# david-cortes/recometrics

Hardware: AMD Instinct MI355X
Metric: users/sec evaluated (all metrics, K=10) (higher is better)
Workload: dtype f32

## Files before the change

### recometrics_amd/_binding.py

```python
import ctypes as C
import os

import numpy as np

_LIB_PATH = os.environ.get("RECOMETRICS_HIP_LIB") or os.path.join(
    os.path.dirname(os.path.abspath(__file__)), "csrc", "librecometrics_hip.so")
_lib = None

METRIC_ORDER = ("p", "tp", "r", "ap", "tap", "ndcg", "hit", "rr", "roc", "pr")
OUTPUTS = tuple(name + ("_auc" if name in ("roc", "pr") else "_at_k") for name in METRIC_ORDER)

_vp, _i32, _i64, _u64, _sz, _ci = C.c_void_p, C.c_int32, C.c_int64, C.c_uint64, C.c_size_t, C.c_int
_FACTORS = (("A", _vp), ("lda", _sz), ("B", _vp), ("ldb", _sz), ("m", _i32), ("n", _i32), ("k", _i32))
_SCORES = (("S", _vp), ("lds", _sz), ("m", _i32), ("n", _i32))


def _csr(which, host, values=False):
    return ((("X%s_csr_p" % which, _vp), ("X%s_csr_i" % which, _vp)) + ((("X%s_csr" % which, _vp),) if values else ())
            + (() if host else (("nnz_" + which, _i64),)))


def _metrics(source, host):
    return (source + _csr("train", host) + _csr("test", host, values=True) + (("k_metrics", _i32), ("cumulative", _ci))
            + ((("break_ties_with_noise", _ci),) if source is _FACTORS else ()) + tuple((name, _vp) for name in OUTPUTS)
# ... 15 lines not shown
                       ("seed", _u64), ("result", C.POINTER(_vp)))}
_TYPED.update({"rm_" + request + source + form: pieces(params, host) for request, pieces in (("calc_metrics", _metrics), ("recommend", _lists))
               for source, params in (("", _FACTORS), ("_scores", _SCORES)) for form, host in (("", True), ("_dev", False))})
SIGNATURES = {name + suffix: (params, _ci) for name, params in _TYPED.items() for suffix in ("_f32", "_f64")}
SIGNATURES.update({
    "rm_has_openmp": ((), _ci), "rm_last_error": ((), C.c_char_p), "rm_device_count": ((), _ci), "rm_set_device": ((("device", _ci),), _ci),
    "rm_set_devices": ((("devices", C.POINTER(_i32)), ("n", _i32)), _ci), "rm_get_devices": ((("devices", C.POINTER(_i32)), ("cap", _i32)), _ci),
    "rm_request_interrupt": ((), None), "rm_get_timings": ((("out", C.POINTER(C.c_double)), ("n", _ci)), _ci), "rm_release_workspace": ((), _ci),
    "rm_debug_reload_switches": ((), None), "rm_debug_sweep_variants": ((("elem_bytes", _ci), ("out", C.POINTER(_ci)), ("cap", _ci)), _ci),
    "rm_debug_find_sweep": (tuple((name, _ci) for name in ("elem_bytes", "ng", "ngt", "auc", "dump", "lmode", "nsub", "spec"))
                            + (("out6", C.POINTER(_ci)),), _ci),
    "rm_debug_supported_ng": ((("elem_bytes", _ci), ("k", _ci)), _ci),
    "rm_debug_sweep_launched": ((("elem_bytes", _ci), ("counts", C.POINTER(_ci)), ("cap", _ci)), _ci), "rm_debug_sweep_launched_reset": ((), None),
    "rm_split_size": ((("result", _vp), ("which", _ci)), _i64), "rm_split_copy": ((("result", _vp), ("which", _ci), ("dst", _vp)), _ci),
    "rm_split_free": ((("result", _vp),), None), "rm_split_last_error": ((), C.c_char_p),
    "rm_csr_rows_sorted": ((("indptr", _vp), ("indices", _vp), ("m", _i32), ("nthreads", _i32)), _ci),
    "rm_csr_sort_rows": ((("indptr", _vp), ("indices", _vp), ("values", _vp), ("value_bytes", _i32), ("m", _i32), ("nthreads", _i32)), _ci),
})
EXPORTS = tuple(SIGNATURES)
HALF_KINDS = ("f16", "bf16")
HALF_SIGNATURES = {"rm_" + request + "_scores" + form + "_" + kind: (pieces(_SCORES, host), _ci)
                   for request, pieces in (("calc_metrics", _metrics), ("recommend", _lists)) for form, host in (("", True), ("_dev", False))
                   for kind in HALF_KINDS}
TEST_HOOKS = {"rm_debug_set_list_ids": ((("ids", C.POINTER(_i32)), ("m", _i32), ("K", _i32)), _ci)}


class HipLibraryMissing(ImportError):
    pass


def lib_path():
    return _LIB_PATH


def _declare(lib, names, table=None):
    for name in names:
        params, restype = (table or SIGNATURES)[name]
        fn = getattr(lib, name)
        fn.argtypes, fn.restype = [ctype for _, ctype in params], restype
    return lib


def load():
    global _lib
    if _lib is None:
        if not os.path.exists(_LIB_PATH):
            raise HipLibraryMissing(
# ... 91 lines not shown


def timings():
    lib = load()
    buf = (C.c_double * 11)()
    n = lib.rm_get_timings(buf, 11)
    keys = ("prep_ms", "sweep_ms", "finalize_ms", "device_ms", "sweep_launches", "item_splits", "sweep_blocks", "lds_bytes",
            "timed_slots", "total_slots", "split_reused")
    return {k: buf[i] for i, k in enumerate(keys[:n])}


def hinted_users():
    lib = load()
    buf = (C.c_double * 12)()
    return int(buf[11]) if lib.rm_get_timings(buf, 12) >= 12 else 0


def set_list_ids(ids):
    lib = load()
    ids = np.ascontiguousarray(ids, dtype=np.int32)
    rc = lib.rm_debug_set_list_ids(ids.ctypes.data_as(C.POINTER(_i32)), ids.shape[0], ids.shape[1])
    if rc:
        _raise(lib, rc)


def csr_rows_sorted(indptr, indices, nthreads=0):
    lib = _load_split()
    assert indptr.dtype == np.int32 and indices.dtype == np.int32
    rc = lib.rm_csr_rows_sorted(_p(indptr), _p(indices), indptr.shape[0] - 1, int(nthreads))
    if rc < 0:
        raise ValueError("rm_csr_rows_sorted: bad argument")
    return bool(rc)


def csr_sort_rows(indptr, indices, data, nthreads=0):
    lib = _load_split()
    assert indptr.dtype == np.int32 and indices.dtype == np.int32 and indices.flags.writeable
    vb = 0 if data is None else data.dtype.itemsize
    if vb not in (0, 4, 8):
        raise ValueError("values must be 4 or 8 bytes wide")
    rc = lib.rm_csr_sort_rows(_p(indptr), _p(indices), None if data is None else _p(data), vb, indptr.shape[0] - 1, int(nthreads))
    if rc:
        raise (MemoryError if rc == 3 else ValueError)("rm_csr_sort_rows failed (status %d)" % rc)


def _invoke(entry, dtype, **values):
# ... 181 lines not shown
```

### recometrics_amd/csrc/rm_device.hpp

```cpp
#pragma once
#include <hip/hip_runtime.h>
#include <stdint.h>

namespace rm {

constexpr int WAVE = 64;
constexpr int GROUP_USERS = 32;
constexpr int TILE_ITEMS = 64;
constexpr int SWEEP_THREADS = 512;
constexpr int GROUPS_PER_BLOCK = 4;
constexpr int POS_CHUNK = 63;
constexpr int MAX_J = 6;
constexpr int STREAM_CLASS = MAX_J + 1;
constexpr int N_CLASSES = MAX_J + 2;
constexpr int IDX_EMPTY = 0x7fffffff;
constexpr int HEAVY_NPOS = 256;
enum : int { LM_LDS = 0, LM_HBM = 1, LM_HBM_APPEND = 2 };
constexpr int WAIT_VMCNT0 = 0x0F70;

enum : int { UF_NAN = 1, UF_ONLY_NDCG = 2, UF_KLEQN = 4, UF_ACTIVE = 8, UF_SKIP = 16 };

enum : int { RQ_P = 1, RQ_TP = 2, RQ_R = 4, RQ_AP = 8, RQ_TAP = 16, RQ_NDCG = 32, RQ_HIT = 64, RQ_RR = 128, RQ_ROC = 256, RQ_PR = 512 };

template <class T> struct Entry { T s; int idx; };
typedef Entry<float> ListEntry;

template <class T> struct PartialStat {
    T vmax, vmin;
    unsigned long long rocsum;
    int has_nan; int pad;
};

struct Plan {
    int n_active;
    int n_slots;
    int n_groups;
    int jmax;
// ... 61 lines not shown
```

### recometrics_amd/csrc/rm_finalize.hpp

```cpp
#pragma once
#include "rm_device.hpp"
#include "rm_kernel_units.hpp"
#include <type_traits>

namespace rm {

constexpr int MAX_PARTS = 128;
constexpr int FIN_THREADS = 128;
constexpr int FIN_TOPV = 64;
template <class T> inline size_t finalize_lds_bytes(int K, int n_part) { return (sizeof(T) * (size_t)(K < FIN_TOPV ? K : FIN_TOPV) + 4 * (size_t)n_part) * FIN_THREADS; }

struct AucPart { unsigned long long sum_ranks; double s1, s2; int nvalid, pad; };

template <class T, class S> struct FinalArgs {
    int m, n, K, n_part, req, cumulative, noise, gu, n_slots;
    const int *slot_user, *slot_chunk;
    const int *train_p, *test_p, *test_i; const T *test_v;
    const int *flags, *user_nslots, *uslot_base, *slot_index;
    const int *gj; const long long *grow;
    const Entry<S> *pl; const PartialStat<S> *pst; const unsigned *hist; const S *pos_score;
    const int *pos_item_tab;
    AucPart *auc_part;
    T *heavy_topv;
    unsigned char *heavy_nan;
// ... 105 lines not shown
                const int pos = filled + __popcll(mk & ((1ull << lane) - 1ull));
                if (cand && pos < K) { L[pos].s = x; L[pos].idx = PI[i]; }
                filled += __popcll(mk);
            }
        }
    }
    #pragma unroll
    for (int d = 32; d >= 1; d >>= 1) {
        const S om = __shfl_xor(vmax, d), on = __shfl_xor(vmin, d);
        vmax = om > vmax ? om : vmax; vmin = on < vmin ? on : vmin;
        has_nan |= __shfl_xor(has_nan, d);
    }
    for (int i = (filled < K ? filled : K) + lane; i < K; i += WAVE) { L[i].s = -(S)INFINITY; L[i].idx = IDX_EMPTY; }
    if (lane == 0) {
        PartialStat<S> ps;
        ps.vmax = vmax; ps.vmin = vmin; ps.rocsum = 0; ps.has_nan = has_nan; ps.pad = 0;
        ((PartialStat<S> *)a.pst)[(size_t)slot * NP + extra] = ps;
    }
}

constexpr int STREAM_RANK_THREADS = 256;
constexpr int STREAM_RANK_ITEMS = 128;
constexpr int STREAM_RANK_LDS = 20 * 1024;
template <class S, int ILP, int LV>
__device__ __forceinline__ void rank_streamed_lds(const S *row, long long i0, int ipt, int n, const int *pit, int P, int top_rt, int lgsb_rt,
                                                  unsigned tab_addr, unsigned hist_addr)
{
    const int top = LV ? (1 << LV) : top_rt;
    const int lgsb = LV ? 14 - LV : lgsb_rt;
    typedef __attribute__((address_space(3))) const S *LdsS;
    typedef __attribute__((address_space(3))) unsigned *LdsU;
    const unsigned sb = 1u << lgsb;
    auto load_batch = [&](int it, S (&x)[ILP]) {
        #pragma unroll
        for (int q = 0; q < ILP; q++) {
            const long long item = i0 + (long long)(it + q) * STREAM_RANK_THREADS + threadIdx.x;
            x[q] = row[item < n ? item : n - 1];
        }
    };
    S nxt[ILP];
    load_batch(0, nxt);
    for (int it = 0; it < ipt; it += ILP) {
        S v[ILP]; unsigned o[ILP];
        #pragma unroll
        for (int q = 0; q < ILP; q++) {
            const long long item = i0 + (long long)(it + q) * STREAM_RANK_THREADS + threadIdx.x;
// ... 42 lines not shown
        const S ps = live ? a.spos_score[te0 + j] : (S)0;
        const bool valid = live && !(isinf(ps) && ps > 0);
        const unsigned long long vm = __ballot(valid);
        const unsigned long long rank = above + incl + 1;
        const int myidx = nvalid + __popcll(vm & ((1ull << lane) - 1ull)) + 1;
        const double term = valid ? (double)myidx / (double)rank : 0.;
        unsigned long long rs = valid ? rank : 0ull;
        #pragma unroll
        for (int dd = 32; dd >= 1; dd >>= 1) {
            const unsigned lo32 = (unsigned)__shfl_xor((int)(unsigned)rs, dd), hi32 = (unsigned)__shfl_xor((int)(unsigned)(rs >> 32), dd);
            rs += ((unsigned long long)hi32 << 32) | lo32;
        }
        sum_ranks += rs;
        for (unsigned long long mm = vm; mm; mm &= mm - 1) s2 += lane_bcast<double>(term, __ffsll((long long)mm) - 1);
        if (a.rank_sorted && valid) a.rank_sorted[te0 + j] = (long long)rank;
        const int last = (base < WAVE ? base : WAVE) - 1;
        above += ((unsigned long long)(unsigned)__shfl((int)(unsigned)(incl >> 32), last) << 32) | (unsigned)__shfl((int)(unsigned)incl, last);
        nvalid += __popcll(vm);
    }
    if (lane == 0) { AucPart r; r.sum_ranks = sum_ranks; r.s1 = 0; r.s2 = s2; r.nvalid = nvalid; r.pad = 0; a.auc_part[slot] = r; }
}

template <class S>
__device__ __forceinline__ bool rank_block_walks(int fused_auc, int P)
{
    if (!(fused_auc & 1)) return false;
    constexpr int per = (int)sizeof(S) / 4;
    int top = 1;
    while (top <= P) top <<= 1;
    return (long long)top * per + P + 1 <= STREAM_RANK_LDS / 4;
}

#define RM_FCMP_LT(m, p, x) asm volatile("v_cmp_lt_f32 %0, %1, %2" : "=s"(m) : "v"(p), "v"(x))
#define RM_FCMP_LT_S(m, p, x) asm volatile("v_cmp_lt_f32 %0, %1, %2" : "=s"(m) : "s"(p), "v"(x))
#define RM_FSEL(d, a, b, m) asm volatile("v_cndmask_b32 %0, %1, %2, %3" : "=v"(d) : "v"(a), "v"(b), "s"(m))
template <int LV>
__device__ __forceinline__ void rank_streamed_fast(const float *row, int i0, int iters, const int *pit, int P, unsigned tab_addr, unsigned hist0_addr,
                                                   float piv_lo, float piv_root, float piv_hi)
{
    constexpr int ILP = 8;
    constexpr int LGSB = 14 - LV;
    constexpr unsigned SB = 1u << LGSB;
    constexpr unsigned Q = SB << (LV - 2);
    typedef __attribute__((address_space(3))) const float *LdsS;
    const float *src = row + i0 + (int)threadIdx.x;
    float nxt[ILP];
    #pragma unroll
    for (int q = 0; q < ILP; q++) nxt[q] = src[q * STREAM_RANK_THREADS];
    const unsigned a1 = tab_addr | Q, a2 = tab_addr | (2 * Q), a3 = tab_addr | (3 * Q);
    for (int it = 0; it < iters; it += ILP) {
        float v[ILP]; unsigned at[ILP];
        #pragma unroll
        for (int q = 0; q < ILP; q++) { v[q] = nxt[q]; at[q] = tab_addr; }
        src += ILP * STREAM_RANK_THREADS;
        if (it + ILP < iters) {
            #pragma unroll
            for (int q = 0; q < ILP; q++) nxt[q] = src[q * STREAM_RANK_THREADS];
        }
        unsigned long long mk0, mk1, mk2;
        #pragma unroll
        for (int i = 0; i < 3 * ILP + 2; i++) {
            if (i < 3 * ILP) {
                const float pv = i < ILP ? piv_lo : (i < 2 * ILP ? piv_root : piv_hi);
                if (i % 3 == 0) RM_FCMP_LT_S(mk0, pv, v[i % ILP]); else if (i % 3 == 1) RM_FCMP_LT_S(mk1, pv, v[i % ILP]); else RM_FCMP_LT_S(mk2, pv, v[i % ILP]);
// ... 27 lines not shown
        #pragma unroll
        for (int q = 0; q < ILP; q++) tie |= nx[q] == v[q];
        if (__any(tie)) {
            #pragma unroll
            for (int q = 0; q < ILP; q++) {
                if (nx[q] == v[q]) {
                    const int item = i0 + (it + q) * STREAM_RANK_THREADS + (int)threadIdx.x;
                    int l = (int)((at[q] - tab_addr) >> LGSB);
                    while (l < P && *(LdsS)(tab_addr + ((unsigned)l << LGSB)) == v[q] && pit[l] > item) l++;
                    at[q] = tab_addr + ((unsigned)l << LGSB);
                }
            }
        }
        const unsigned one = 1u;
        #pragma unroll
        for (int q = 0; q < ILP; q++) {
            const unsigned ha = hist0_addr + (((at[q] - tab_addr) >> LGSB) << 2);
            asm volatile("ds_add_u32 %0, %1" :: "v"(ha), "v"(one) : "memory");
        }
    }
    __builtin_amdgcn_s_waitcnt(0xC07F);
}

template <class T, class S>
__global__ __launch_bounds__(STREAM_RANK_THREADS) void k_rank_streamed(FinalArgs<T, S> a, int parts, int ipt, int row0)
{
    __shared__ __attribute__((aligned(16384))) char rk_smem[STREAM_RANK_LDS];
    const int d = row0 + blockIdx.x / parts, part = blockIdx.x % parts;
    const int slot = a.stream_slot0 + d;
    const int u = a.slot_user[slot];
    if (a.flags[u] & UF_ONLY_NDCG) return;
    const int te0 = a.test_p[u], P = a.test_p[u + 1] - te0;
    constexpr int WORDS = STREAM_RANK_LDS / 4;
    constexpr int per = (int)sizeof(S) / 4;
    int top = 1;
    while (top <= P) top <<= 1;
    int R = 0;
    if ((long long)top * per + P + 1 <= WORDS) { R = 1; while (R < 32 && (long long)top * 2 * R * per + P + 1 <= WORDS) R *= 2; }
    const int *pit = a.spos_item + te0;
    const S *row = a.stream_scores + (size_t)d * (size_t)a.stream_ld;
    const long long i0 = (long long)part * STREAM_RANK_THREADS * ipt;
    if (R > 0) {
        S *lds_s = (S *)rk_smem;
        unsigned *lds_h = (unsigned *)(rk_smem + sizeof(S) * (size_t)top * (size_t)R) + 1;
        for (int i = threadIdx.x; i < top * R; i += STREAM_RANK_THREADS) { const int e = i / R; lds_s[i] = e < P ? a.spos_score[te0 + e] : (S)INFINITY; }
        for (int i = threadIdx.x; i < P; i += STREAM_RANK_THREADS) lds_h[i] = 0u;
        __syncthreads();
        int lgsb = sizeof(S) == 4 ? 2 : 3;
        for (int r = R; r > 1; r >>= 1) lgsb++;
        const unsigned tab_addr = (unsigned)(size_t)(__attribute__((address_space(3))) char *)rk_smem + (unsigned)((threadIdx.x & (R - 1)) * sizeof(S));
        const unsigned hist_addr = (unsigned)(size_t)(__attribute__((address_space(3))) char *)lds_h;
        const bool full = (long long)top * R == 4096 / per;
        if (sizeof(S) == 4 && full && top >= 128 && top <= 1024 && !a.rank_generic) {
            const int inside = (int)((a.n - i0) / STREAM_RANK_THREADS);
            const int iters = inside <= 0 ? 0 : (inside < ipt ? inside : ipt) / 8 * 8;
            if (iters > 0) {
                const float *tabf = (const float *)lds_s;
                const float p_lo = tabf[(top / 4 - 1) * R], p_root = tabf[(top / 2 - 1) * R], p_hi = tabf[(3 * top / 4 - 1) * R];
                const float s_lo = __builtin_bit_cast(float, __builtin_amdgcn_readfirstlane(__builtin_bit_cast(int, p_lo)));
                const float s_root = __builtin_bit_cast(float, __builtin_amdgcn_readfirstlane(__builtin_bit_cast(int, p_root)));
                const float s_hi = __builtin_bit_cast(float, __builtin_amdgcn_readfirstlane(__builtin_bit_cast(int, p_hi)));
                const float *rowf = (const float *)row;
                const unsigned h0 = hist_addr - 4u;
                if (top == 128) rank_streamed_fast<7>(rowf, (int)i0, iters, pit, P, tab_addr, h0, s_lo, s_root, s_hi);
                else if (top == 256) rank_streamed_fast<8>(rowf, (int)i0, iters, pit, P, tab_addr, h0, s_lo, s_root, s_hi);
                else if (top == 512) rank_streamed_fast<9>(rowf, (int)i0, iters, pit, P, tab_addr, h0, s_lo, s_root, s_hi);
                else rank_streamed_fast<10>(rowf, (int)i0, iters, pit, P, tab_addr, h0, s_lo, s_root, s_hi);
            }
            if (iters < ipt) rank_streamed_lds<S, 8, 0>(row, i0 + (long long)iters * STREAM_RANK_THREADS, ipt - iters, a.n, pit, P, top, lgsb, tab_addr, hist_addr);
        } else
        if (full && top == 128) rank_streamed_lds<S, 8, 7>(row, i0, ipt, a.n, pit, P, top, lgsb, tab_addr, hist_addr);
        else if (full && top == 256) rank_streamed_lds<S, 8, 8>(row, i0, ipt, a.n, pit, P, top, lgsb, tab_addr, hist_addr);
        else if (full && top == 512) rank_streamed_lds<S, 8, 9>(row, i0, ipt, a.n, pit, P, top, lgsb, tab_addr, hist_addr);
        else if (full && top == 1024) rank_streamed_lds<S, 8, 10>(row, i0, ipt, a.n, pit, P, top, lgsb, tab_addr, hist_addr);
        else rank_streamed_lds<S, 8, 0>(row, i0, ipt, a.n, pit, P, top, lgsb, tab_addr, hist_addr);
        __syncthreads();
        if (parts == 1 && (a.fused_auc & 1)) {
            if (threadIdx.x < WAVE) {
                const bool own = (a.fused_auc & 2) != 0;
                const S *sp = a.spos_score + te0;
                auc_walk_streamed<T, S>(a, slot, te0, P, (int)threadIdx.x, [&](int j) {
                    unsigned c = lds_h[j];
                    if (own && j + 1 < P) { const S x = sp[j + 1]; c += (!(isinf(x) && x > 0) && x == x) ? 1u : 0u; }
                    return c;
                });
            }
            return;
        }
        for (int i = threadIdx.x; i < P; i += STREAM_RANK_THREADS) { const unsigned c = lds_h[i]; if (c) atomicAdd(&a.shist[te0 + i], c); }
    } else {
// ... 797 lines not shown
```

### recometrics_amd/csrc/rm_lib.hip

```cpp
#include <hip/hip_runtime.h>

#include <algorithm>
#include <array>
#include <cmath>
#include <cstdio>
#include <cstring>
#include <cstdlib>
#include <type_traits>
#include <atomic>
#include <chrono>
#include <condition_variable>
#include <csignal>
#include <functional>
#include <limits>
#include <map>
#include <memory>
#include <mutex>
#include <string>
#include <thread>
#include <vector>

#include "../../include/recometrics_hip.h"
#include "../../include/recometrics_hip_half.h"
#include "rm_device.hpp"
// ... 1024 lines not shown
            side.await(SIDE_CHECKS_DONE, stream); pos.await(POS_MAXIMA_DONE, stream);
            HIP_CHECK(hipMemcpyAsync(cx.pinned_plan, plan, sizeof(Plan), hipMemcpyDeviceToHost, stream));
            if (attempt == 0 && flat_early) {
                const hipStream_t sc = pos.fork(POS_SCORES_AFTER_COPY);
                if (c.scores) {
                    hipLaunchKernelGGL(k_test_masked, dim3(cdiv(m, TM_USERS)), dim3(256), 0, sc, m, c.test_p, c.test_i, c.train_p, c.train_i, ent_user, ent_masked, plan);
                    with_score_src<T>(c.s_type, [&](auto *src) {
                        typedef std::remove_cv_t<std::remove_pointer_t<decltype(src)>> Src;
                        hipLaunchKernelGGL((k_pos_scores_given<T, Src>), dim3(cdiv(c.nnz_test, 256)), dim3(256), 0, sc, pf, (const Src *)c.S, c.lds, (const int *)ent_user, (const unsigned char *)ent_masked);
                    });
                } else {
                hipLaunchKernelGGL(k_pos_scores_flat<T>, dim3(cdiv(c.nnz_test, POSF_WAVES * WAVE)), dim3(POSF_WAVES * WAVE), 0, sc, pf, ent_user);
                if (masked_from_bits) side.await(SIDE_ROWS_FOR_POS, sc);
                else hipLaunchKernelGGL(k_test_masked, dim3(cdiv(m, TM_USERS)), dim3(256), 0, sc, m, c.test_p, c.test_i, c.train_p, c.train_i, ent_user, ent_masked, plan);
                hipLaunchKernelGGL(k_pos_apply_masked<T>, dim3(cdiv(c.nnz_test, 256)), dim3(256), 0, sc, pf, ent_masked);
                }
                pos.mark(POS_SCORES_DONE);
            }
            RM_TRACE_POINT("run: plan chain + side kernels enqueued");
            HIP_CHECK(hipStreamSynchronize(stream));
            RM_TRACE_POINT("run: plan read back");
            hp = *cx.pinned_plan;
            throw_csr_defects(hp, c, cx);
            if (ca.allow_stream && !ca.force_stream && hp.class_count[STREAM_CLASS] > stream_cap && attempt == 0) {
                ca.allow_stream = 0; ca.check_ptr = 0; keepable = false;
                side.sync(); pos.sync();
                continue;
            }
            break;
        }
        if (!reused) throw_csr_defects(hp, c, cx);
        n_slots = hp.n_slots;
        n_stream = (want_auc || ext_topk) ? hp.class_count[STREAM_CLASS] : 0;
        stream_slot0 = n_stream > 0 ? hp.class_offset[STREAM_CLASS] : n_slots;
        if (!reused) check_nan = scores_may_overflow();
    }
    bool scores_may_overflow()
    {
        if (items_known) { hp.amax_b = cx.packed.amax_b; hp.nonfinite_b = cx.packed.nonfinite_b; }
        else { cx.packed.amax_b = hp.amax_b; cx.packed.nonfinite_b = hp.nonfinite_b; }
        double amax_a, amax_b;
        std::memcpy(&amax_a, &hp.amax_a, 8); std::memcpy(&amax_b, &hp.amax_b, 8);
        const double tmax = std::is_same<T, float>::value ? 3.0e38 : 1.0e308;
        if (c.scores) return false;
        return hp.nonfinite || hp.nonfinite_b || !((double)k * amax_a * 1.001 < tmax / std::max(amax_b, 1e-300));
    }

    bool make_split_key(SplitKey &key) const
    {
        std::memset(&key, 0, sizeof(SplitKey));
        if (g_sw.no_split_cache || !use_side || c.reco || c.scores || !c.plain() || c.items_tag != 0 || !c.test_p || m <= 0) return false;
        const void *arr[SPLIT_ARRAYS] = {c.train_p, c.train_i, c.test_p, c.test_i, c.test_v};
        const long long words[SPLIT_ARRAYS] = {(long long)m + 1, std::max<long long>(c.nnz_train, 0), (long long)m + 1, std::max<long long>(c.nnz_test, 0),
                                               c.test_v ? std::max<long long>(c.nnz_test, 0) * (long long)(sizeof(T) / 4) : 0};
        long long total = 0;
        for (int i = 0; i < SPLIT_ARRAYS; i++) { key.arr[i] = arr[i]; key.words[i] = words[i]; total += words[i]; }
// ... 301 lines not shown
    }

    void topk_rows()
    {
        HIP_CHECK(hipEventRecord(cx.ev[EV_PREP_END], stream));
        const void *kernel = nullptr;
        with_score_src<T>(c.s_type, [&](auto *src) {
            typedef std::remove_cv_t<std::remove_pointer_t<decltype(src)>> Src;
            RowTopkArgs<T, Src> ra{n, K, c.train_p, c.train_i, (const Src *)c.S, c.lds, c.topk_idx, c.topk_score, c.status};
            hipLaunchKernelGGL((k_topk_rows<T, Src>), dim3((unsigned)m), dim3(SCORE_ROW_THREADS), 0, stream, ra);
            kernel = (const void *)k_topk_rows<T, Src>;
        });
        HIP_CHECK(hipGetLastError());
        RM_TRACE_POINT("run: row top-K enqueued");
        HIP_CHECK(hipEventRecord(cx.ev[EV_SWEEP_END], stream));
        double *tm = cx.timings;
        hipFuncAttributes at{};
        HIP_CHECK(hipFuncGetAttributes(&at, kernel));
        tm[4] = 1; tm[5] = 1; tm[6] = m; tm[7] = (double)at.sharedSizeBytes;
        cx.timed_slots = hp.n_slots; cx.total_slots = hp.n_slots;
    }

    int stream_parts() const { return (int)cdiv(n, STREAM_RANK_THREADS * STREAM_RANK_ITEMS); }
    void rank_streamed_rows(int r0, int r1, hipStream_t st)
    {
        if (r1 <= r0) return;
        const int parts = stream_parts();
        const int ipt = ((int)cdiv(n, (long long)parts * STREAM_RANK_THREADS) + 7) / 8 * 8;
        hipLaunchKernelGGL((k_rank_streamed<T, T>), dim3((unsigned)((long long)(r1 - r0) * parts)), dim3(STREAM_RANK_THREADS), 0, st, fa, parts, ipt, r0);
    }
    void auc_streamed_rows(int r0, int r1, hipStream_t st)
    {
        if (r1 <= r0) return;
        hipLaunchKernelGGL((k_auc_streamed<T, T>), dim3(cdiv((long long)(r1 - r0) * WAVE, 256)), dim3(256), 0, st, fa, r0, r1);
    }
    void finalize_slots(int s0, int s1, size_t fin_lds)
    {
        if (s1 <= s0) return;
        fa.fin_slot0 = s0; fa.fin_slot1 = s1;
        hipLaunchKernelGGL((k_finalize<T, T>), dim3(cdiv(s1 - s0, FIN_THREADS)), dim3(FIN_THREADS), fin_lds, stream, fa);
    }

    void collect_lists()
    {
        if (!collect) return;
        fa.collected = 1;
        const char *gl = (const char *)glists;
        if (collect_capw(K, collect_g.lane_cap) == 512)
            hipLaunchKernelGGL((k_collect_topk<T, T, ThrT, 512>), dim3(collect_grid(cdiv(n_slots, 4))), dim3(256), 0, stream, fa, collect_g, gl, lane_cnt, (const ThrT *)thr_shared);
        else if (collect_capw(K, collect_g.lane_cap) == 1024)
            hipLaunchKernelGGL((k_collect_topk<T, T, ThrT, 1024>), dim3(collect_grid(cdiv(n_slots, 4))), dim3(256), 0, stream, fa, collect_g, gl, lane_cnt, (const ThrT *)thr_shared);
        else
// ... 15 lines not shown
        fa.n_part = g.n_part; fa.pl = pl; fa.pst = pst;
        fa.stream_slot0 = stream_slot0; fa.stream_scores = stream_scores; fa.stream_ld = stream_ld;
        collect_lists();
        select_lists();
        const bool merged_ready = n_slots > 0 && (collect || ext_topk);
        RecoArgs<T> ra{m, n, K, g.n_part, flags, uslot_base, slot_index, c.train_p, pl, pst, merged_ready ? merged : nullptr,
                       c.topk_idx, c.topk_score, c.status};
        const size_t lds = reco_lds_bytes<T>(g.n_part, merged_ready);
        if (lds > 48 * 1024) HIP_CHECK(hipFuncSetAttribute((const void *)k_finalize_reco<T>, hipFuncAttributeMaxDynamicSharedMemorySize, (int)lds));
        hipLaunchKernelGGL(k_finalize_reco<T>, dim3(cdiv(m, RECO_THREADS)), dim3(RECO_THREADS), lds, stream, ra);
        HIP_CHECK(hipGetLastError());
    }

    void finalize()
    {
        fa.n_part = g.n_part; fa.pl = pl; fa.pst = pst; fa.hist = hist; fa.pos_score = pos_score; fa.pos_item_tab = pos_item;
        fa.stream_slot0 = stream_slot0; fa.stream_scores = stream_scores; fa.stream_ld = stream_ld;
        fa.spos_score = spos_score; fa.spos_item = spos_item; fa.shist = shist;
        fa.rank_generic = (g_sw.rank_generic ? 1 : 0);
        const bool ranks_beside = use_side && n_slots > 0 && want_auc && n_stream > 0;
        bool auc_launch = true;
        if (stream_parts() == 1 && !g_sw.no_fused_auc) {
            fa.fused_auc = 1 | (g.mask_test ? 2 : 0);
            long long top = 1;
            while (top <= hp.max_npos) top <<= 1;
            auc_launch = ext_topk || !(top * (long long)(sizeof(T) / 4) + hp.max_npos + 1 <= STREAM_RANK_LDS / 4);
        }
        hipStream_t rank_stream = stream;
        if (ranks_beside) { rank_stream = side.fork(SIDE_FORK); rank_streamed_rows(0, n_stream, rank_stream); }
        if (g.mask_test) {
            if (n_slots > stream_slot0)
                hipLaunchKernelGGL((k_merge_positives<T, T>), dim3(cdiv(n_slots - stream_slot0, MERGE_WAVES)), dim3(MERGE_WAVES * WAVE), 0, stream, fa, g.n_part - 1, stream_slot0);
            if (ranks_beside && auc_launch) rank_stream = side.fork(SIDE_MERGED);
        }
        if (ranks_beside && auc_launch) auc_streamed_rows(0, n_stream, rank_stream);
        hipLaunchKernelGGL((k_finalize_skipped<T, T>), dim3(cdiv(m, 256)), dim3(256), 0, stream, fa);
        if (side.marked(SIDE_TOP_VALUES)) side.await(SIDE_TOP_VALUES, stream);
        collect_lists();
        select_lists();
        if (n_slots > 0) {
            if (want_auc) {
                if (n_stream > 0 && !ranks_beside) { rank_streamed_rows(0, n_stream, stream); if (auc_launch) auc_streamed_rows(0, n_stream, stream); }
                if (stream_slot0 > 0) hipLaunchKernelGGL((k_auc_slots<T, T>), dim3(cdiv(stream_slot0, 256)), dim3(256), 0, stream, fa);
            }
            const size_t fin_lds = finalize_lds_bytes<T>(K, g.n_part);
            HIP_CHECK(hipFuncSetAttribute((const void *)k_finalize<T, T>, hipFuncAttributeMaxDynamicSharedMemorySize, (int)fin_lds));
            fa.auc_defer_slot0 = n_slots;
            if (ranks_beside && (req & (RQ_ROC | RQ_PR)) && !g_sw.no_defer_auc) {
                fa.auc_defer_slot0 = stream_slot0;
                finalize_slots(0, n_slots, fin_lds);
                side.join(SIDE_JOIN);
                hipLaunchKernelGGL((k_finalize_auc<T, T>), dim3(cdiv(n_slots - stream_slot0, 256)), dim3(256), 0, stream, fa);
            } else if (ranks_beside) {
                finalize_slots(0, stream_slot0, fin_lds);
                side.join(SIDE_JOIN);
                finalize_slots(stream_slot0, n_slots, fin_lds);
            } else finalize_slots(0, n_slots, fin_lds);
        }
        HIP_CHECK(hipGetLastError());
    }

    void export_ranks()
    {
        if (c.topk_idx && !c.reco)
            hipLaunchKernelGGL(k_export_rank<T>, dim3(cdiv((long long)m * K, 256)), dim3(256), 0, stream, m, K, merged, c.topk_idx, c.topk_score, flags);
// ... 1254 lines not shown
{
    return elem_bytes == 4   ? debug_find_sweep<SweepArgs>(ng, ngt, auc, dump, lmode, nsub, spec, out6)
           : elem_bytes == 8 ? debug_find_sweep<Sweep64Args>(ng, ngt, auc, dump, lmode, nsub, spec, out6) : -1;
}
extern "C" int rm_debug_supported_ng(int elem_bytes, int k)
{
    return elem_bytes == 4 ? Prec<float>::supported_ng(k) : elem_bytes == 8 ? Prec<double>::supported_ng(k) : -1;
}
template <class Args> int debug_sweep_launched(int *counts, int cap)
{
    const int n = debug_sweep_variants<Args>(nullptr, 0);
    for (int i = 0; counts && i < n && i < cap; i++) counts[i] = i < LEDGER_ROWS ? sweep_ledger<Args>()[i].load(std::memory_order_relaxed) : 0;
    return n;
}
extern "C" int rm_debug_sweep_launched(int elem_bytes, int *counts, int cap)
{
    return elem_bytes == 4 ? debug_sweep_launched<SweepArgs>(counts, cap) : elem_bytes == 8 ? debug_sweep_launched<Sweep64Args>(counts, cap) : -1;
}
extern "C" void rm_debug_sweep_launched_reset(void)
{
    for (auto &prec : g_sweep_launched) for (auto &c : prec) c.store(0, std::memory_order_relaxed);
}

template <class T> __global__ void k_set_list_ids(long long count, Entry<T> *lists, const int *ids)
{
    const long long i = (long long)blockIdx.x * blockDim.x + threadIdx.x;
    if (i < count) lists[i].idx = ids[i];
}
extern "C" int rm_debug_set_list_ids(const int32_t *ids, int32_t m, int32_t K)
{
    return guarded([&] {
        Ctx &cx = context(0);
        std::lock_guard<std::mutex> lk(cx.mu);
        const SplitCache &kept = cx.split;
        const Workspace::Buf buf = cx.ws.peek(WS_MERGED);
        const long long count = (long long)m * K;
        if (!ids || m <= 0 || K <= 0 || !kept.valid || !kept.lists.current(cx.ws) || kept.key.m != m || kept.key.K != K ||
            (size_t)count * (kept.key.elem == 4 ? sizeof(Entry<float>) : sizeof(Entry<double>)) > buf.bytes)
            throw RmError{RM_ERR_INVALID, "rm_debug_set_list_ids: the context keeps no lists of " + std::to_string(m) + " x " + std::to_string(K) + " entries"};
        HIP_CHECK(hipDeviceSynchronize());
        int *dev = nullptr;
        HIP_CHECK(hipMalloc((void **)&dev, sizeof(int) * (size_t)count));
        hipError_t e = hipMemcpy(dev, ids, sizeof(int) * (size_t)count, hipMemcpyHostToDevice);
        if (e == hipSuccess) {
            if (kept.key.elem == 4) hipLaunchKernelGGL(k_set_list_ids<float>, dim3(cdiv(count, 256)), dim3(256), 0, nullptr, count, (Entry<float> *)buf.ptr, (const int *)dev);
            else hipLaunchKernelGGL(k_set_list_ids<double>, dim3(cdiv(count, 256)), dim3(256), 0, nullptr, count, (Entry<double> *)buf.ptr, (const int *)dev);
// ... 44 lines not shown
```

### recometrics_amd/csrc/rm_prep.hpp

```cpp
#pragma once
#include "rm_device.hpp"
#include "rm_kernel_units.hpp"

namespace rm {

struct ClassifyArgs {
    int m, n, K;
    const int *train_p, *test_p;
    int req;
    int cold, min_items_pool, min_pos_test;
    int want_auc;
    int *flags;
    int *user_nslots;
    int *heavy_users;
    Plan *plan;
    const unsigned char *only;
    int force_stream;
    int allow_stream;
    int check_ptr;
    int heavy_npos;
    long long nnz_train, nnz_test;
    int reco;
};

// ... 92 lines not shown
    const bool skip = u < a.m && a.only && !a.only[u];
    bool live = u < a.m && !skip;
    if (skip) { a.flags[u] = UF_SKIP; a.user_nslots[u] = 0; }
    int ntr = 0, npos = 0;
    if (live) {
        const int a0 = a.train_p[u], a1 = a.train_p[u + 1], b0 = a.reco ? 0 : a.test_p[u], b1 = a.reco ? 0 : a.test_p[u + 1];
        if (a.check_ptr && (a0 < 0 || a1 < a0 || (long long)a1 > a.nnz_train || b0 < 0 || b1 < b0 || (long long)b1 > a.nnz_test)) {
            atomicOr(&a.plan->csr_bad, CSR_BAD_INDPTR); a.plan->csr_where = u;
        } else { ntr = a1 - a0; npos = b1 - b0; }
    }
    const int cand = a.n - ntr;
    bool isnan_user = !live || npos <= 0 || (ntr + npos >= a.n && !(a.req & RQ_NDCG)) || cand < a.min_items_pool ||
                      (!a.cold && ntr == 0) || npos < a.min_pos_test;
    if (a.reco) isnan_user = !live || cand < 1;
    const bool only_ndcg = !a.reco && (ntr + npos) >= a.n;
    const bool kleqn = cand <= a.K;
    if (!a.reco && !isnan_user && kleqn && !(a.req & (RQ_ROC | RQ_PR | RQ_AP | RQ_TAP | RQ_RR))) isnan_user = true;
    int f = 0, nsl = 0, myclass = -1, nfull = 0;
    if (isnan_user) f = UF_NAN;
    else {
        f = UF_ACTIVE | (only_ndcg ? UF_ONLY_NDCG : 0) | (kleqn ? UF_KLEQN : 0);
        if (a.force_stream || (a.want_auc && !only_ndcg && npos > POS_CHUNK && a.allow_stream)) {
            nsl = 1;
            myclass = STREAM_CLASS;
        } else if (a.want_auc && !only_ndcg) {
            nfull = npos / POS_CHUNK;
            const int rem = npos % POS_CHUNK;
            nsl = nfull + (rem ? 1 : 0);
            myclass = rem ? chunk_depth(rem) : -1;
        } else {
            nsl = 1;
            myclass = 0;
        }
    }
    __shared__ int blk_count[N_CLASSES + 3];
    __shared__ int blk_heavy[2];
    if (threadIdx.x < N_CLASSES + 3) blk_count[threadIdx.x] = 0;
    if (threadIdx.x < 2) blk_heavy[threadIdx.x] = 0;
    __syncthreads();
    const int lane = threadIdx.x & 63;
    const unsigned long long act = __ballot(!isnan_user);
    if (act && lane == __ffsll((long long)act) - 1) atomicAdd(&blk_count[N_CLASSES], __popcll(act));
    for (int j = 0; j < N_CLASSES; j++) {
        const unsigned long long mk = __ballot(myclass == j);
        if (mk && lane == __ffsll((long long)mk) - 1) atomicAdd(&blk_count[j], __popcll(mk));
    }
    if (nfull) atomicAdd(&blk_count[MAX_J], nfull);
// ... 99 lines not shown
};

constexpr int ASSIGN_THREADS = 1024;
__global__ __launch_bounds__(ASSIGN_THREADS) void k_assign_slots(AssignArgs a)
#ifdef RM_PREP_PLAIN_KERNELS
{
    __shared__ int blk_count[N_CLASSES], blk_base[N_CLASSES], blk_chunks, blk_chunk_base;
    if (a.plan->csr_bad & CSR_BAD_INDPTR) return;
    const int u = blockIdx.x * blockDim.x + threadIdx.x;
    const int lane = threadIdx.x & 63;
    if (threadIdx.x < N_CLASSES) blk_count[threadIdx.x] = 0;
    if (threadIdx.x == N_CLASSES) blk_chunks = 0;
    __syncthreads();
    const int nsl = u < a.m ? a.user_nslots[u] : 0;
    const int npos = (nsl && a.test_p) ? a.test_p[u + 1] - a.test_p[u] : 0;
    int ubase = 0;
    if (u < a.m) {
        ubase = a.uslot_base[u] + (a.tile_offset ? a.tile_offset[u >> 10] : 0);
        if (a.tile_offset) ((int *)a.uslot_base)[u] = ubase;
    }
    const bool auc_user = nsl && a.want_auc && !(a.flags[u] & UF_ONLY_NDCG);
    int jlast = -1, in_blk = 0;
    const bool streamed = nsl && (a.force_stream || (auc_user && nsl == 1 && npos > POS_CHUNK));
    if (nsl) jlast = streamed ? STREAM_CLASS : auc_user ? chunk_depth(min(POS_CHUNK, npos - (nsl - 1) * POS_CHUNK)) : 0;
    for (int j = 0; j < N_CLASSES; j++) {
        const unsigned long long mk = __ballot(jlast == j);
        if (!mk) continue;
        const int leader = __ffsll((long long)mk) - 1;
        int base = 0;
        if (lane == leader) base = atomicAdd(&blk_count[j], __popcll(mk));
        base = __shfl(base, leader);
        if (jlast == j) in_blk = base + __popcll(mk & ((1ull << lane) - 1));
    }
    int full_at = 0;
    if (nsl > 1) full_at = atomicAdd(&blk_count[MAX_J], nsl - 1);
    const int nch = (streamed && auc_user) ? (npos + POS_CHUNK - 1) / POS_CHUNK : 0;
    int ch_at = 0;
    if (nch) ch_at = atomicAdd(&blk_chunks, nch);
    __syncthreads();
    if (threadIdx.x < N_CLASSES && blk_count[threadIdx.x]) blk_base[threadIdx.x] = atomicAdd(&a.plan->class_cursor[threadIdx.x], blk_count[threadIdx.x]);
    if (threadIdx.x == N_CLASSES && blk_chunks) blk_chunk_base = atomicAdd(&a.plan->n_stream_chunks, blk_chunks);
    __syncthreads();
    if (nch) {
        const int at = blk_chunk_base + ch_at;
        for (int c = 0; c < nch; c++) { a.sc_user[at + c] = u; a.sc_chunk[at + c] = c; }
    }
    if (nsl) {
// ... 13 lines not shown
}
#else
;
#endif

__global__ __launch_bounds__(1024) void k_block_tables(Plan *p, const unsigned char *slot_j, int *gj, long long *grow, int gu)
#ifdef RM_PREP_PLAIN_KERNELS
{
    __shared__ int wsum[16];
    __shared__ long long carry_s;
    if (p->csr_bad & CSR_BAD_INDPTR) return;
    const int tid = threadIdx.x, lane = tid & 63, wave = __builtin_amdgcn_readfirstlane(tid >> 6);
    const int ng = p->n_groups, ns = p->n_slots;
    const int nb = (ng + GROUPS_PER_BLOCK - 1) / GROUPS_PER_BLOCK;
    if (tid == 0) carry_s = 0;
    __syncthreads();
    for (int base = 0; base < nb; base += 1024) {
        const int b = base + tid;
        int jb = 0, ngb = 0;
        if (b < nb) {
            const int glast = min(ng, (b + 1) * GROUPS_PER_BLOCK) - 1;
            const int slast = min(ns, (glast + 1) * gu) - 1;
            jb = slot_j[slast];
            if (jb == STREAM_CLASS) {
                const int first_stream = p->class_offset[STREAM_CLASS];
                jb = first_stream > b * GROUPS_PER_BLOCK * gu ? slot_j[first_stream - 1] : 0;
            }
            ngb = glast - b * GROUPS_PER_BLOCK + 1;
        }
        const int per_group = (1 << jb) - 1;
        const int v = ngb * per_group;
        int x = v;
        #pragma unroll
        for (int d = 1; d < 64; d <<= 1) { const int y = __shfl_up(x, d); if (lane >= d) x += y; }
        if (lane == 63) wsum[wave] = x;
        __syncthreads();
        int woff = 0;
        for (int w = 0; w < wave; w++) woff += wsum[w];
        const long long carry = carry_s;
        const long long mine = carry + woff + x - v;
        for (int q = 0; q < ngb; q++) {
            const int g = b * GROUPS_PER_BLOCK + q;
            gj[g] = jb;
            grow[g] = mine + (long long)q * per_group;
        }
        __syncthreads();
        if (tid == 1023) carry_s = carry + woff + x;
// ... 860 lines not shown
```

Before: 19.79 million.

## Split streamed users into size classes and size rank-table LDS per class

Streamed users are binned into several classes by their positive count, and the rank kernel is launched per group of classes with dynamic LDS sized for that class. An optional compile-time switch lets the 256–1024 entry tables use a wider per-copy layout so the fast rank routine can serve them with more LDS. With the switch at its default of zero, every class keeps the same 20KB LDS, so all classes merge into one launch over the sorted rows. The risks are extra launches, extra plan classes to scan in prep, and a possible alignment mismatch with dynamic shared memory that makes the fast path fall back.

```diff
diff --git a/recometrics_amd/_binding.py b/recometrics_amd/_binding.py
--- a/recometrics_amd/_binding.py
+++ b/recometrics_amd/_binding.py
@@ -61,7 +61,8 @@
 HALF_SIGNATURES = {"rm_" + request + "_scores" + form + "_" + kind: (pieces(_SCORES, host), _ci)
                    for request, pieces in (("calc_metrics", _metrics), ("recommend", _lists)) for form, host in (("", True), ("_dev", False))
                    for kind in HALF_KINDS}
-TEST_HOOKS = {"rm_debug_set_list_ids": ((("ids", C.POINTER(_i32)), ("m", _i32), ("K", _i32)), _ci)}
+TEST_HOOKS = {"rm_debug_set_list_ids": ((("ids", C.POINTER(_i32)), ("m", _i32), ("K", _i32)), _ci),
+              "rm_debug_rank_table": ((("P", _i32), ("elem_bytes", _i32), ("out7", C.POINTER(_i32))), _ci)}
 
 
 class HipLibraryMissing(ImportError):
@@ -199,6 +200,14 @@
     rc = lib.rm_debug_set_list_ids(ids.ctypes.data_as(C.POINTER(_i32)), ids.shape[0], ids.shape[1])
     if rc:
         _raise(lib, rc)
+
+
+def rank_table(npos, elem_bytes=4):
+    buf = (_i32 * 7)()
+    if load().rm_debug_rank_table(npos, elem_bytes, buf):
+        raise ValueError("rm_debug_rank_table(%r, %r)" % (npos, elem_bytes))
+    keys = ("entries", "copies", "used_bytes", "lds_bytes", "launch_lds_bytes", "block_walks", "host_fits")
+    return dict(zip(keys, (int(x) for x in buf)))
 
 
 def csr_rows_sorted(indptr, indices, nthreads=0):
diff --git a/recometrics_amd/csrc/rm_device.hpp b/recometrics_amd/csrc/rm_device.hpp
--- a/recometrics_amd/csrc/rm_device.hpp
+++ b/recometrics_amd/csrc/rm_device.hpp
@@ -12,7 +12,15 @@
 constexpr int POS_CHUNK = 63;
 constexpr int MAX_J = 6;
 constexpr int STREAM_CLASS = MAX_J + 1;
-constexpr int N_CLASSES = MAX_J + 2;
+constexpr int STREAM_CLASSES = 5;
+constexpr int N_CLASSES = MAX_J + 1 + STREAM_CLASSES;
+__host__ __device__ inline int stream_class_top(int c) { return c == 0 ? 0 : 2048 >> c; }
+__host__ __device__ inline int stream_class_of(int npos)
+{
+    int c = STREAM_CLASSES - 1;
+    while (c > 0 && npos >= stream_class_top(c)) c--;
+    return STREAM_CLASS + c;
+}
 constexpr int IDX_EMPTY = 0x7fffffff;
 constexpr int HEAVY_NPOS = 256;
 enum : int { LM_LDS = 0, LM_HBM = 1, LM_HBM_APPEND = 2 };
diff --git a/recometrics_amd/csrc/rm_finalize.hpp b/recometrics_amd/csrc/rm_finalize.hpp
--- a/recometrics_amd/csrc/rm_finalize.hpp
+++ b/recometrics_amd/csrc/rm_finalize.hpp
@@ -151,6 +151,27 @@
 constexpr int STREAM_RANK_THREADS = 256;
 constexpr int STREAM_RANK_ITEMS = 128;
 constexpr int STREAM_RANK_LDS = 20 * 1024;
+#ifndef RM_RANK_WIDE_TOPS
+#define RM_RANK_WIDE_TOPS 0
+#endif
+constexpr int RANK_WIDE_TOPS = RM_RANK_WIDE_TOPS;
+__host__ __device__ inline int rank_table_top(int P) { int top = 1; while (top <= P) top <<= 1; return top; }
+__host__ __device__ inline int rank_lds_bytes(int top, int per)
+{
+    if (per == 1 && (top & RANK_WIDE_TOPS)) return top * 32 * 4 + (top + 1) * 4;
+    return STREAM_RANK_LDS;
+}
+__host__ __device__ inline int rank_class_lds_bytes(int sc, int per) { return rank_lds_bytes(stream_class_top(sc) ? stream_class_top(sc) : 2048, per); }
+__host__ __device__ inline int rank_table_copies(int P, int per)
+{
+    const int top = rank_table_top(P);
+    const long long words = rank_lds_bytes(top, per) / 4;
+    if (!((long long)top * per + P + 1 <= words)) return 0;
+    int R = 1;
+    while (R < 32 && (long long)top * 2 * R * per + P + 1 <= words) R *= 2;
+    return R;
+}
+__host__ __device__ inline bool rank_table_fits(int P, int per) { return rank_table_copies(P, per) > 0; }
 template <class S, int ILP, int LV>
 __device__ __forceinline__ void rank_streamed_lds(const S *row, long long i0, int ipt, int n, const int *pit, int P, int top_rt, int lgsb_rt,
                                                   unsigned tab_addr, unsigned hist_addr)
@@ -239,24 +260,19 @@
 }
 
 template <class S>
-__device__ __forceinline__ bool rank_block_walks(int fused_auc, int P)
-{
-    if (!(fused_auc & 1)) return false;
-    constexpr int per = (int)sizeof(S) / 4;
-    int top = 1;
-    while (top <= P) top <<= 1;
-    return (long long)top * per + P + 1 <= STREAM_RANK_LDS / 4;
+__host__ __device__ __forceinline__ bool rank_block_walks(int fused_auc, int P)
+{
+    return (fused_auc & 1) && rank_table_fits(P, (int)sizeof(S) / 4);
 }
 
 #define RM_FCMP_LT(m, p, x) asm volatile("v_cmp_lt_f32 %0, %1, %2" : "=s"(m) : "v"(p), "v"(x))
 #define RM_FCMP_LT_S(m, p, x) asm volatile("v_cmp_lt_f32 %0, %1, %2" : "=s"(m) : "s"(p), "v"(x))
 #define RM_FSEL(d, a, b, m) asm volatile("v_cndmask_b32 %0, %1, %2, %3" : "=v"(d) : "v"(a), "v"(b), "s"(m))
-template <int LV>
+template <int LV, int LGSB>
 __device__ __forceinline__ void rank_streamed_fast(const float *row, int i0, int iters, const int *pit, int P, unsigned tab_addr, unsigned hist0_addr,
                                                    float piv_lo, float piv_root, float piv_hi)
 {
     constexpr int ILP = 8;
-    constexpr int LGSB = 14 - LV;
     constexpr unsigned SB = 1u << LGSB;
     constexpr unsigned Q = SB << (LV - 2);
     typedef __attribute__((address_space(3))) const float *LdsS;
@@ -330,21 +346,21 @@
     __builtin_amdgcn_s_waitcnt(0xC07F);
 }
 
+constexpr int rank_fast_lgsb(int lv) { return (lv == 7 || ((RANK_WIDE_TOPS >> lv) & 1)) ? 7 : 14 - lv; }
+static_assert((RANK_WIDE_TOPS & ~(256 | 512 | 1024)) == 0, "wide tables: the depths the fast routine serves beyond 128 entries");
+
 template <class T, class S>
 __global__ __launch_bounds__(STREAM_RANK_THREADS) void k_rank_streamed(FinalArgs<T, S> a, int parts, int ipt, int row0)
 {
-    __shared__ __attribute__((aligned(16384))) char rk_smem[STREAM_RANK_LDS];
+    extern __shared__ __attribute__((aligned(16))) char rk_smem[];
     const int d = row0 + blockIdx.x / parts, part = blockIdx.x % parts;
     const int slot = a.stream_slot0 + d;
     const int u = a.slot_user[slot];
     if (a.flags[u] & UF_ONLY_NDCG) return;
     const int te0 = a.test_p[u], P = a.test_p[u + 1] - te0;
-    constexpr int WORDS = STREAM_RANK_LDS / 4;
     constexpr int per = (int)sizeof(S) / 4;
-    int top = 1;
-    while (top <= P) top <<= 1;
-    int R = 0;
-    if ((long long)top * per + P + 1 <= WORDS) { R = 1; while (R < 32 && (long long)top * 2 * R * per + P + 1 <= WORDS) R *= 2; }
+    const int top = rank_table_top(P);
+    const int R = rank_table_copies(P, per);
     const int *pit = a.spos_item + te0;
     const S *row = a.stream_scores + (size_t)d * (size_t)a.stream_ld;
     const long long i0 = (long long)part * STREAM_RANK_THREADS * ipt;
@@ -356,10 +372,12 @@
         __syncthreads();
         int lgsb = sizeof(S) == 4 ? 2 : 3;
         for (int r = R; r > 1; r >>= 1) lgsb++;
-        const unsigned tab_addr = (unsigned)(size_t)(__attribute__((address_space(3))) char *)rk_smem + (unsigned)((threadIdx.x & (R - 1)) * sizeof(S));
+        const unsigned smem_addr = (unsigned)(size_t)(__attribute__((address_space(3))) char *)rk_smem;
+        const unsigned tab_addr = smem_addr + (unsigned)((threadIdx.x & (R - 1)) * sizeof(S));
         const unsigned hist_addr = (unsigned)(size_t)(__attribute__((address_space(3))) char *)lds_h;
         const bool full = (long long)top * R == 4096 / per;
-        if (sizeof(S) == 4 && full && top >= 128 && top <= 1024 && !a.rank_generic) {
+        const int lgsb_fast = top == 128 ? rank_fast_lgsb(7) : top == 256 ? rank_fast_lgsb(8) : top == 512 ? rank_fast_lgsb(9) : top == 1024 ? rank_fast_lgsb(10) : -1;
+        if (sizeof(S) == 4 && lgsb == lgsb_fast && !(smem_addr & (((unsigned)top << lgsb) - 1u)) && !a.rank_generic) {
             const int inside = (int)((a.n - i0) / STREAM_RANK_THREADS);
             const int iters = inside <= 0 ? 0 : (inside < ipt ? inside : ipt) / 8 * 8;
             if (iters > 0) {
@@ -370,10 +388,10 @@
                 const float s_hi = __builtin_bit_cast(float, __builtin_amdgcn_readfirstlane(__builtin_bit_cast(int, p_hi)));
                 const float *rowf = (const float *)row;
                 const unsigned h0 = hist_addr - 4u;
-                if (top == 128) rank_streamed_fast<7>(rowf, (int)i0, iters, pit, P, tab_addr, h0, s_lo, s_root, s_hi);
-                else if (top == 256) rank_streamed_fast<8>(rowf, (int)i0, iters, pit, P, tab_addr, h0, s_lo, s_root, s_hi);
-                else if (top == 512) rank_streamed_fast<9>(rowf, (int)i0, iters, pit, P, tab_addr, h0, s_lo, s_root, s_hi);
-                else rank_streamed_fast<10>(rowf, (int)i0, iters, pit, P, tab_addr, h0, s_lo, s_root, s_hi);
+                if (top == 128) rank_streamed_fast<7, rank_fast_lgsb(7)>(rowf, (int)i0, iters, pit, P, tab_addr, h0, s_lo, s_root, s_hi);
+                else if (top == 256) rank_streamed_fast<8, rank_fast_lgsb(8)>(rowf, (int)i0, iters, pit, P, tab_addr, h0, s_lo, s_root, s_hi);
+                else if (top == 512) rank_streamed_fast<9, rank_fast_lgsb(9)>(rowf, (int)i0, iters, pit, P, tab_addr, h0, s_lo, s_root, s_hi);
+                else rank_streamed_fast<10, rank_fast_lgsb(10)>(rowf, (int)i0, iters, pit, P, tab_addr, h0, s_lo, s_root, s_hi);
             }
             if (iters < ipt) rank_streamed_lds<S, 8, 0>(row, i0 + (long long)iters * STREAM_RANK_THREADS, ipt - iters, a.n, pit, P, top, lgsb, tab_addr, hist_addr);
         } else
diff --git a/recometrics_amd/csrc/rm_lib.hip b/recometrics_amd/csrc/rm_lib.hip
--- a/recometrics_amd/csrc/rm_lib.hip
+++ b/recometrics_amd/csrc/rm_lib.hip
@@ -1070,7 +1070,7 @@
             RM_TRACE_POINT("run: plan read back");
             hp = *cx.pinned_plan;
             throw_csr_defects(hp, c, cx);
-            if (ca.allow_stream && !ca.force_stream && hp.class_count[STREAM_CLASS] > stream_cap && attempt == 0) {
+            if (ca.allow_stream && !ca.force_stream && hp.class_offset[N_CLASSES] - hp.class_offset[STREAM_CLASS] > stream_cap && attempt == 0) {
                 ca.allow_stream = 0; ca.check_ptr = 0; keepable = false;
                 side.sync(); pos.sync();
                 continue;
@@ -1079,7 +1079,7 @@
         }
         if (!reused) throw_csr_defects(hp, c, cx);
         n_slots = hp.n_slots;
-        n_stream = (want_auc || ext_topk) ? hp.class_count[STREAM_CLASS] : 0;
+        n_stream = (want_auc || ext_topk) ? hp.class_offset[N_CLASSES] - hp.class_offset[STREAM_CLASS] : 0;
         stream_slot0 = n_stream > 0 ? hp.class_offset[STREAM_CLASS] : n_slots;
         if (!reused) check_nan = scores_may_overflow();
     }
@@ -1427,12 +1427,26 @@
     }
 
     int stream_parts() const { return (int)cdiv(n, STREAM_RANK_THREADS * STREAM_RANK_ITEMS); }
-    void rank_streamed_rows(int r0, int r1, hipStream_t st)
+    void rank_streamed_rows(int r0, int r1, int lds, hipStream_t st)
     {
         if (r1 <= r0) return;
         const int parts = stream_parts();
         const int ipt = ((int)cdiv(n, (long long)parts * STREAM_RANK_THREADS) + 7) / 8 * 8;
-        hipLaunchKernelGGL((k_rank_streamed<T, T>), dim3((unsigned)((long long)(r1 - r0) * parts)), dim3(STREAM_RANK_THREADS), 0, st, fa, parts, ipt, r0);
+        if (lds > 48 * 1024) HIP_CHECK(hipFuncSetAttribute((const void *)k_rank_streamed<T, T>, hipFuncAttributeMaxDynamicSharedMemorySize, lds));
+        hipLaunchKernelGGL((k_rank_streamed<T, T>), dim3((unsigned)((long long)(r1 - r0) * parts)), dim3(STREAM_RANK_THREADS), (size_t)lds, st, fa, parts, ipt, r0);
+    }
+    void rank_streamed_all(hipStream_t st)
+    {
+        const int per = (int)sizeof(T) / 4;
+        auto class_lds = [&](int sc) { return rank_class_lds_bytes(sc, per); };
+        for (int sc = 0; sc < STREAM_CLASSES; ) {
+            int last = sc;
+#ifndef RM_RANK_LAUNCH_PER_CLASS
+            while (last + 1 < STREAM_CLASSES && class_lds(last + 1) == class_lds(sc)) last++;
+#endif
+            rank_streamed_rows(hp.class_offset[STREAM_CLASS + sc] - stream_slot0, hp.class_offset[STREAM_CLASS + last + 1] - stream_slot0, class_lds(sc), st);
+            sc = last + 1;
+        }
     }
     void auc_streamed_rows(int r0, int r1, hipStream_t st)
     {
@@ -1494,12 +1508,10 @@
         bool auc_launch = true;
         if (stream_parts() == 1 && !g_sw.no_fused_auc) {
             fa.fused_auc = 1 | (g.mask_test ? 2 : 0);
-            long long top = 1;
-            while (top <= hp.max_npos) top <<= 1;
-            auc_launch = ext_topk || !(top * (long long)(sizeof(T) / 4) + hp.max_npos + 1 <= STREAM_RANK_LDS / 4);
+            auc_launch = ext_topk || !rank_table_fits(hp.max_npos, (int)sizeof(T) / 4);
         }
         hipStream_t rank_stream = stream;
-        if (ranks_beside) { rank_stream = side.fork(SIDE_FORK); rank_streamed_rows(0, n_stream, rank_stream); }
+        if (ranks_beside) { rank_stream = side.fork(SIDE_FORK); rank_streamed_all(rank_stream); }
         if (g.mask_test) {
             if (n_slots > stream_slot0)
                 hipLaunchKernelGGL((k_merge_positives<T, T>), dim3(cdiv(n_slots - stream_slot0, MERGE_WAVES)), dim3(MERGE_WAVES * WAVE), 0, stream, fa, g.n_part - 1, stream_slot0);
@@ -1512,7 +1524,7 @@
         select_lists();
         if (n_slots > 0) {
             if (want_auc) {
-                if (n_stream > 0 && !ranks_beside) { rank_streamed_rows(0, n_stream, stream); if (auc_launch) auc_streamed_rows(0, n_stream, stream); }
+                if (n_stream > 0 && !ranks_beside) { rank_streamed_all(stream); if (auc_launch) auc_streamed_rows(0, n_stream, stream); }
                 if (stream_slot0 > 0) hipLaunchKernelGGL((k_auc_slots<T, T>), dim3(cdiv(stream_slot0, 256)), dim3(256), 0, stream, fa);
             }
             const size_t fin_lds = finalize_lds_bytes<T>(K, g.n_part);
@@ -2813,6 +2825,19 @@
     for (auto &prec : g_sweep_launched) for (auto &c : prec) c.store(0, std::memory_order_relaxed);
 }
 
+extern "C" int rm_debug_rank_table(int32_t P, int32_t elem_bytes, int32_t *out7)
+{
+    if (!out7 || P < 0 || (elem_bytes != 4 && elem_bytes != 8)) return -1;
+    const int per = elem_bytes / 4, top = rank_table_top(P), R = rank_table_copies(P, per);
+    out7[0] = top; out7[1] = R;
+    out7[2] = R > 0 ? top * R * elem_bytes + 4 * (P + 1) : 0;
+    out7[3] = rank_lds_bytes(top, per);
+    out7[4] = rank_class_lds_bytes(stream_class_of(P) - STREAM_CLASS, per);
+    out7[5] = (elem_bytes == 4 ? rank_block_walks<float>(1, P) : rank_block_walks<double>(1, P)) ? 1 : 0;
+    out7[6] = rank_table_fits(P, per) ? 1 : 0;
+    return 0;
+}
+
 template <class T> __global__ void k_set_list_ids(long long count, Entry<T> *lists, const int *ids)
 {
     const long long i = (long long)blockIdx.x * blockDim.x + threadIdx.x;
diff --git a/recometrics_amd/csrc/rm_prep.hpp b/recometrics_amd/csrc/rm_prep.hpp
--- a/recometrics_amd/csrc/rm_prep.hpp
+++ b/recometrics_amd/csrc/rm_prep.hpp
@@ -138,7 +138,7 @@
         f = UF_ACTIVE | (only_ndcg ? UF_ONLY_NDCG : 0) | (kleqn ? UF_KLEQN : 0);
         if (a.force_stream || (a.want_auc && !only_ndcg && npos > POS_CHUNK && a.allow_stream)) {
             nsl = 1;
-            myclass = STREAM_CLASS;
+            myclass = stream_class_of(npos);
         } else if (a.want_auc && !only_ndcg) {
             nfull = npos / POS_CHUNK;
             const int rem = npos % POS_CHUNK;
@@ -284,7 +284,7 @@
     const bool auc_user = nsl && a.want_auc && !(a.flags[u] & UF_ONLY_NDCG);
     int jlast = -1, in_blk = 0;
     const bool streamed = nsl && (a.force_stream || (auc_user && nsl == 1 && npos > POS_CHUNK));
-    if (nsl) jlast = streamed ? STREAM_CLASS : auc_user ? chunk_depth(min(POS_CHUNK, npos - (nsl - 1) * POS_CHUNK)) : 0;
+    if (nsl) jlast = streamed ? stream_class_of(npos) : auc_user ? chunk_depth(min(POS_CHUNK, npos - (nsl - 1) * POS_CHUNK)) : 0;
     for (int j = 0; j < N_CLASSES; j++) {
         const unsigned long long mk = __ballot(jlast == j);
         if (!mk) continue;
@@ -344,7 +344,7 @@
             const int glast = min(ng, (b + 1) * GROUPS_PER_BLOCK) - 1;
             const int slast = min(ns, (glast + 1) * gu) - 1;
             jb = slot_j[slast];
-            if (jb == STREAM_CLASS) {
+            if (jb >= STREAM_CLASS) {
                 const int first_stream = p->class_offset[STREAM_CLASS];
                 jb = first_stream > b * GROUPS_PER_BLOCK * gu ? slot_j[first_stream - 1] : 0;
             }
```

Result: no change. 19.78 million (-0.0%).
